# alvinwan/neural-backed-decision-trees

Measured on AMD Instinct MI355X. Metric: images/sec training SoftNBDT WRN28x10 CIFAR10, higher is better.
Workload: dtype bf16; 1 GPU; WideResNet-28-10 + SoftTreeSupLoss (induced-wrn28_10_cifar10, 10 leaves), CIFAR10-shaped 3x32x32, SGD m=0.9 wd=5e-4; batch_per_gpu=512, global_batch=512, parallelism=dp1

## Files before the change

### include/nbdt_hip.h

```cpp
#ifndef NBDT_HIP_H
#define NBDT_HIP_H

#include <stdint.h>

#ifdef __cplusplus
extern "C" {
#endif

#define NBDT_OK 0
#define NBDT_EINVAL (-1)
#define NBDT_EHIP (-2)
#define NBDT_ENOMEM (-3)

#define NBDT_F32 0
#define NBDT_BF16 1
#define NBDT_F16 2

const char* nbdt_last_error(void);
const char* nbdt_debug_last_igemm(void);
const char* nbdt_debug_last_igemm_full(void);
const char* nbdt_debug_last_wgrad(void);
int nbdt_version(void);
int nbdt_set_deterministic(int32_t on);
int nbdt_get_deterministic(void);
// ... 273 lines not shown
                         int32_t C, float* out, void* stream);
int nbdt_ref_bn_act_bwd(const float* gu, const float* gate, const float* gpool, const float* x, const float* save_mean,
                        const float* save_rstd, const float* gamma, const float* beta, int32_t act, const float* gx_add,
                        int32_t B, int32_t H, int32_t W, int32_t C, float* dsum, float* dgamma, float* dbeta, float* gx,
                        void* stream);
int nbdt_ref_dwconv_fwd(const float* x, const float* w, int32_t B, int32_t H, int32_t W, int32_t C, int32_t k,
                        int32_t stride, float* y, void* stream);
int nbdt_ref_dwconv_bwd_data(const float* gy, const float* w, int32_t B, int32_t H, int32_t W, int32_t C, int32_t k,
                             int32_t stride, float* gx, void* stream);
int nbdt_ref_dwconv_bwd_weight(const float* x, const float* gy, int32_t B, int32_t H, int32_t W, int32_t C, int32_t k,
                               int32_t stride, float* dw, void* stream);

int nbdt_stem_conv(const float* img, const float* w, int32_t B, int32_t H, int32_t W,
                   int32_t cout_real, int32_t cpad, int32_t stride, void* out, void* stream);
int nbdt_stem_wgrad(const float* img, const void* gy, int32_t B, int32_t H, int32_t W,
                    int32_t cout_real, int32_t cpad, int32_t stride, float* dw, void* stream);
int nbdt_linear_fwd(const float* x, const float* w, const float* b, int32_t B, int32_t K, int32_t N,
                    float* z, void* stream);
int nbdt_linear_bwd(const float* x, const float* w, const float* gz, int32_t B, int32_t K, int32_t N,
                    float* gx, float* gw, float* gb, void* stream);
int nbdt_sgd_step(float* p, float* g, float* buf, int64_t n, float lr, float momentum,
                  float weight_decay, float grad_scale, void* p_bf16, int32_t zero_grad, void* stream);

#define NBDT_U8 3
#define NBDT_AUGMENT_MAX_PAD 32
int nbdt_augment_batch(const void* src, int32_t src_dtype, const int64_t* labels_src, const int64_t* index, int32_t B,
                       int64_t N, int32_t H, int32_t W, int32_t pad, int32_t flip, const float* mean, const float* std,
                       const float* fill, uint64_t seed, uint64_t epoch, const int8_t* params_in, float* out,
                       int64_t* labels_out, int8_t* params_out, void* stream);

#define NBDT_RESIZED_CROP_RATIOS 4096
#define NBDT_RESIZED_CROP_ATTEMPTS 10
int nbdt_resized_crop_batch(const void* src, int32_t src_dtype, const int64_t* labels_src, const int64_t* index, int32_t B,
                            int64_t N, int32_t H, int32_t W, int32_t rs_h, int32_t rs_w, int32_t win_top, int32_t win_left,
                            int32_t out_h, int32_t out_w, int32_t flip, const float* mean, const float* std,
                            const double* scale, const double* ratio, const double* ratio_table, uint64_t seed,
                            uint64_t epoch, const int32_t* params_in, float* out, int64_t* labels_out, int32_t* params_out,
                            void* stream);
int nbdt_resized_crop_band_rows(int32_t H, int32_t W, int32_t rs_h, int32_t rs_w, int32_t win_top, int32_t win_left,
                                int32_t out_h, int32_t out_w);

int nbdt_augment_batch_sharded(const void* src, int32_t src_dtype, const int64_t* labels_src, const int64_t* index,
                               int64_t index_base, int32_t B, int64_t N, int32_t H, int32_t W, int32_t pad, int32_t flip,
                               const float* mean, const float* std, const float* fill, uint64_t seed, uint64_t epoch,
                               const int8_t* params_in, float* out, int64_t* labels_out, int8_t* params_out, void* stream);
int nbdt_resized_crop_batch_sharded(const void* src, int32_t src_dtype, const int64_t* labels_src, const int64_t* index,
// ... 26 lines not shown
```

### neural-backed-decision-trees_amd/csrc/common.h

```cpp
#pragma once
#include <hip/hip_runtime.h>
#include <hip/hip_bf16.h>
#include <hip/hip_fp16.h>
#include <stdint.h>
#include <stdio.h>
#include <string.h>

#include <mutex>

#include "../../include/nbdt_hip.h"

#if !defined(NBDT_TIMING_BUILD) &&                                                                                    \
    (defined(NBDT_EPI_TIMING) || (defined(NBDT_PP_TIMING) && (NBDT_PP_TIMING + 0) != 0) ||                            \
     (defined(NBDT_WPP_TIMING) && (NBDT_WPP_TIMING + 0) != 0) || (defined(NBDT_SEG_TIMING) && (NBDT_SEG_TIMING + 0) != 0) || \
     (defined(NBDT_RULES_TIMING) && (NBDT_RULES_TIMING + 0) != 0))
#error "timing switch without -DNBDT_TIMING_BUILD: a stamped build is not a product library (csrc/common.h)"
#endif
#ifdef NBDT_TIMING_BUILD
extern "C" __attribute__((weak, used, visibility("default"))) int nbdt_timing_build() { return 1; }
#endif

namespace nbdt {

extern thread_local char g_err[512];
// ... 43 lines not shown
bool wgrad_store_epilogue();
int reserved_cus();
float* det_rows(hipStream_t st, size_t floats);
const char* det_rows_why();
int det_fold(hipStream_t st, const float* rows, int nrows, size_t n, float* dst);

typedef unsigned short bf16_t;

__device__ __forceinline__ float bf16_to_f32(bf16_t v) {
  return __uint_as_float(((unsigned)v) << 16);
}
__device__ __forceinline__ bf16_t f32_to_bf16(float f) {
  unsigned u = __float_as_uint(f);
  if ((u & 0x7fffffffu) > 0x7f800000u) return (bf16_t)((u >> 16) | 0x40);
  u += 0x7fffu + ((u >> 16) & 1u);
  return (bf16_t)(u >> 16);
}
__device__ __forceinline__ unsigned pack_bf16x2(float lo, float hi) {
  unsigned r;
  asm("v_cvt_pk_bf16_f32 %0, %1, %2" : "=v"(r) : "v"(lo), "v"(hi));
  return r;
}

struct FastDiv {
  unsigned mul, sh, d;
};
inline FastDiv make_fastdiv(unsigned d) {
  FastDiv f;
  f.d = d;
  if (d == 1) { f.mul = 0; f.sh = 0; return f; }
  unsigned s = 0;
  while ((1ull << s) < d) ++s;
  const unsigned long long num = 1ull << (31 + s);
  f.mul = (unsigned)((num + d - 1) / d);
  f.sh = s - 1;
  return f;
}
__device__ __forceinline__ unsigned fdiv(unsigned n, const FastDiv& f) {
  return f.d == 1 ? n : (__umulhi(n, f.mul) >> f.sh);
}

struct PadGeom {
  int B, H, W, C;
  int npix;
  int row;
  int img;
// ... 119 lines not shown
```

### neural-backed-decision-trees_amd/csrc/conv.hip

```cpp
#include "common.h"
#include <stdlib.h>

using namespace nbdt;

static int check_desc(const nbdt_conv_desc* d);

static int conv_igemm_impl(const nbdt_conv_desc* d, const void* in, const void* w, void* out, const void* residual,
                           float* bn_scratch, void* stream, const nbdt::BnBwdArgs* bn = nullptr) {
  NBDT_REQUIRE(d && in && w && out, "null argument");
  int rc = check_desc(d);
  if (rc) return rc;
  const void* res = d->accumulate ? (const void*)out : residual;
  NBDT_REQUIRE(!(d->accumulate && residual), "accumulate and residual are exclusive");
  const int64_t M64 = (int64_t)d->B * d->gh * d->gw;
  NBDT_REQUIRE(M64 < (1ll << 31), "pixel grid too large");
  const int M = (int)M64;
  hipStream_t st = (hipStream_t)stream;
  nbdt::HaloGeom hg;
  if (nbdt::conv_halo_applicable(d, M, &hg))
    return nbdt::conv3x3_halo(d, hg, in, w, out, res, bn_scratch, bn, M, st);
  NBDT_REQUIRE(d->wide_tile != 2 && d->wide_tile != 4 && d->wide_tile != 5,
               "wide_tile = 2 / 4 / 5 (force 512-pixel tiles [with the padded LDS pitch] / half tiles): not a dense 3x3 stride-1 conv it fits");
  nbdt::g_last_igemm = "conv_igemm_dma_kernel";
  return nbdt::conv_igemm_dma(d, in, w, out, res, bn_scratch, bn, M, st);
// ... 72 lines not shown
  return conv_igemm_impl(d, in, w, out, residual, bn_scratch, stream);
}

extern "C" int nbdt_conv_igemm_bnbwd(const nbdt_conv_desc* d, const void* in, const void* w, void* out,
                                     const void* bn_x, const float* save_mean, const float* save_rstd,
                                     const float* gamma, const float* beta, float* bn_partials, void* stream) {
  NBDT_REQUIRE(bn_x && save_mean && save_rstd && gamma && beta && bn_partials, "null BatchNorm argument");
  NBDT_REQUIRE(d && !d->accumulate, "fused BatchNorm-backward sums are for plain outputs");
  nbdt::BnBwdArgs bn{bn_x, save_mean, save_rstd, gamma, beta};
  return conv_igemm_impl(d, in, w, out, nullptr, bn_partials, stream, &bn);
}

extern "C" int nbdt_conv_igemm_affine(const nbdt_conv_desc* d, const void* in, const void* w, void* out,
                                      const void* residual, const float* scale, const float* shift, int32_t act,
                                      void* stream) {
  NBDT_REQUIRE(scale && shift, "null scale / shift");
  NBDT_REQUIRE(act >= 0 && act <= 2, "unknown activation");
  NBDT_REQUIRE(d && !d->accumulate, "the fused inference epilogue is for plain outputs");
  nbdt::BnBwdArgs ep{nullptr, nullptr, nullptr, nullptr, nullptr};
  ep.aff_scale = scale; ep.aff_shift = shift; ep.aff_act = act;
  return conv_igemm_impl(d, in, w, out, residual, nullptr, stream, &ep);
}

__global__ __launch_bounds__(256) void weight_prep_kernel(const float* __restrict__ w, int cout, int taps,
                                                          int cin, bf16_t* __restrict__ wb,
                                                          bf16_t* __restrict__ wd) {
  const int64_t n = (int64_t)cout * taps * cin;
  for (int64_t i = (int64_t)blockIdx.x * 256 + threadIdx.x; i < n; i += (int64_t)gridDim.x * 256) {
    const bf16_t v = f32_to_bf16(w[i]);
    if (wb) wb[i] = v;
    if (wd) {
      const int ci = (int)(i % cin);
      const int64_t r = i / cin;
      const int t = (int)(r % taps);
      const int co = (int)(r / taps);
      wd[((int64_t)ci * taps + (taps - 1 - t)) * cout + co] = v;
    }
  }
}

__global__ __launch_bounds__(256) void weight_prep_batched_kernel(const float* __restrict__ flat,
                                                                  const long long* __restrict__ table, int n_layers,
                                                                  long long total_tiles, bf16_t* __restrict__ wd_flat) {
  __shared__ long long tab[64 * 6];
  __shared__ float tile[64][33];
  for (int i = threadIdx.x; i < n_layers * 6; i += 256) tab[i] = table[i];
  __syncthreads();
  const int tx = threadIdx.x & 31, ty = threadIdx.x >> 5;
  const int wx = threadIdx.x & 63, wy = threadIdx.x >> 6;
  for (long long e = blockIdx.x; e < total_tiles; e += gridDim.x) {
    int l = 0;
    while (l + 1 < n_layers && e >= tab[(l + 1) * 6 + 5]) ++l;
    const long long* T = tab + l * 6;
    const int cout = (int)T[2], taps = (int)T[3], cin = (int)T[4];
    const int cit = cin >> 5, cot = (cout + 63) >> 6;
    long long i = e - T[5];
    const int ci0 = (int)(i % cit) * 32;
    i /= cit;
    const int co0 = (int)(i % cot) * 64;
    const int t = (int)(i / cot);
    const float* src = flat + T[0];
    bf16_t* dst = wd_flat + T[1];
#pragma unroll
    for (int r = ty; r < 64; r += 8)
      tile[r][tx] = co0 + r < cout ? src[((long long)(co0 + r) * taps + t) * cin + ci0 + tx] : 0.f;
    __syncthreads();
#pragma unroll
    for (int r = wy; r < 32; r += 4)
      if (co0 + wx < cout)
        dst[((long long)(ci0 + r) * taps + (taps - 1 - t)) * cout + co0 + wx] = f32_to_bf16(tile[wx][r]);
    __syncthreads();
  }
}

extern "C" int nbdt_weight_prep_batched(const float* flat, const int64_t* table, int32_t n_layers, int64_t total_tiles,
                                        void* wd_flat, void* stream) {
  NBDT_REQUIRE(flat && table && wd_flat, "null argument");
  NBDT_REQUIRE(n_layers > 0 && n_layers <= 64 && total_tiles > 0, "bad layer table");
  long long blocks = total_tiles < 8192 ? total_tiles : 8192;
  hipLaunchKernelGGL(weight_prep_batched_kernel, dim3((unsigned)blocks), dim3(256), 0, (hipStream_t)stream, flat,
                     (const long long*)table, n_layers, (long long)total_tiles, (bf16_t*)wd_flat);
  NBDT_LAUNCH_CHECK();
  return NBDT_OK;
}

__global__ __launch_bounds__(256) void weight_tile_batched_kernel(const bf16_t* __restrict__ src,
                                                                  const long long* __restrict__ table, int n,
                                                                  long long total_tiles, bf16_t* __restrict__ dst) {
  __shared__ long long tab[64 * 5];
  for (int i = threadIdx.x; i < n * 5; i += 256) tab[i] = table[i];
  __syncthreads();
  for (long long e = blockIdx.x; e < total_tiles; e += gridDim.x) {
    int l = 0;
    while (l + 1 < n && e >= tab[(l + 1) * 5 + 4]) ++l;
    const long long* T = tab + l * 5;
    const int rows = (int)T[2], k = (int)T[3];
    const int nt32 = rows / 32;
    const int nt = nt32 % 5 == 0 ? 5 : (nt32 % 4 == 0 ? 4 : (nt32 % 2 == 0 ? 2 : 1));
    const int bn = 32 * nt, kchunks = k / 32;
    long long i = e - T[4];
    const int tap = (int)(i % 9);
    i /= 9;
    const int kc = (int)(i % kchunks);
    const int n_blk = (int)(i / kchunks);
    const bf16_t* s0 = src + T[0];
    bf16_t* d0 = dst + T[1] + (e - T[4]) * (long long)(bn * 32);
    for (int q = threadIdx.x; q < bn * 4; q += 256) {
      const int r = q >> 2, cp = q & 3;
      const int c = cp ^ ((r >> 2) & 3);
      const u32x4_t v = *(const u32x4_t*)(s0 + ((long long)(n_blk * bn + r) * 9 + tap) * k + kc * 32 + c * 8);
      *(u32x4_t*)(d0 + r * 32 + cp * 8) = v;
    }
  }
}

extern "C" int nbdt_weight_tile_batched(const void* src_bf16, const int64_t* table, int32_t n, int64_t total_tiles,
                                        void* dst_bf16, void* stream) {
  NBDT_REQUIRE(src_bf16 && table && dst_bf16, "null argument");
  NBDT_REQUIRE(n > 0 && n <= 64 && total_tiles > 0, "bad matrix table");
  long long blocks = total_tiles < 8192 ? total_tiles : 8192;
  hipLaunchKernelGGL(weight_tile_batched_kernel, dim3((unsigned)blocks), dim3(256), 0, (hipStream_t)stream,
                     (const bf16_t*)src_bf16, (const long long*)table, n, (long long)total_tiles, (bf16_t*)dst_bf16);
  NBDT_LAUNCH_CHECK();
  return NBDT_OK;
}

extern "C" int nbdt_weight_prep(const float* w, int32_t cout, int32_t taps, int32_t cin, void* w_bf16,
                                void* wd_bf16, void* stream) {
  NBDT_REQUIRE(w && (w_bf16 || wd_bf16), "null argument");
  NBDT_REQUIRE(cout > 0 && taps > 0 && cin > 0, "bad shape");
  const int64_t n = (int64_t)cout * taps * cin;
  const int grid = (int)((n + 255) / 256 < 2048 ? (n + 255) / 256 : 2048);
  hipLaunchKernelGGL(weight_prep_kernel, dim3(grid), dim3(256), 0, (hipStream_t)stream, w, cout, taps, cin,
                     (bf16_t*)w_bf16, (bf16_t*)wd_bf16);
  NBDT_LAUNCH_CHECK();
  return NBDT_OK;
}
```

### neural-backed-decision-trees_amd/csrc/misc.hip

```cpp
#include "common.h"

#include <atomic>
#include <map>
#include <utility>

using namespace nbdt;

namespace nbdt {
static std::atomic<int> g_deterministic{0};
bool deterministic() { return g_deterministic.load(std::memory_order_relaxed) != 0; }

struct DetBuf { float* ptr = nullptr; size_t floats = 0; bool captured = false; };
static std::mutex g_det_mutex;
static std::map<std::pair<int, hipStream_t>, DetBuf> g_det_bufs;

static thread_local char g_det_why[200] = "";
const char* det_rows_why() { return g_det_why; }

float* det_rows(hipStream_t st, size_t floats) {
  int dev = 0;
  snprintf(g_det_why, sizeof(g_det_why), "hipMalloc / hipGetDevice failed");
  if (hipGetDevice(&dev) != hipSuccess) return nullptr;
  std::lock_guard<std::mutex> lock(g_det_mutex);
  DetBuf& b = g_det_bufs[std::make_pair(dev, st)];
// ... 468 lines not shown
    const long long n = (long long)B * K;
    hipLaunchKernelGGL(linear_bwd_x_kernel, dim3((unsigned)((n + 255) / 256)), dim3(256), 0, st, gz, w, B, K, N, gx);
    NBDT_LAUNCH_CHECK();
  }
  if (gw) {
    const long long n = (long long)N * (K + 1);
    const int splits = (B >= 64 && !deterministic()) ? 16 : 1;
    const int bpb = (B + splits - 1) / splits;
    hipLaunchKernelGGL(linear_bwd_w_kernel, dim3((unsigned)((n + 255) / 256), (B + bpb - 1) / bpb), dim3(256), 0, st, gz,
                       x, B, K, N, bpb, gw, gb);
    NBDT_LAUNCH_CHECK();
  }
  return NBDT_OK;
}

__global__ __launch_bounds__(256) void sgd_kernel(float* __restrict__ p, float* __restrict__ g,
                                                  float* __restrict__ buf, long long n, float lr, float momentum,
                                                  float wd, float gscale, bf16_t* __restrict__ pb, int zero_g) {
  const long long n4 = n >> 2;
  for (long long i = (long long)blockIdx.x * 256 + threadIdx.x; i < n4; i += (long long)gridDim.x * 256) {
    float4 pv = ((const float4*)p)[i];
    const float4 gv = ((const float4*)g)[i];
    float4 bv = ((const float4*)buf)[i];
    bv.x = momentum * bv.x + (gscale * gv.x + wd * pv.x);
    bv.y = momentum * bv.y + (gscale * gv.y + wd * pv.y);
    bv.z = momentum * bv.z + (gscale * gv.z + wd * pv.z);
    bv.w = momentum * bv.w + (gscale * gv.w + wd * pv.w);
    pv.x -= lr * bv.x; pv.y -= lr * bv.y; pv.z -= lr * bv.z; pv.w -= lr * bv.w;
    ((float4*)buf)[i] = bv;
    ((float4*)p)[i] = pv;
    if (zero_g) ((float4*)g)[i] = float4{0.f, 0.f, 0.f, 0.f};
    if (pb) {
      uint2 o;
      o.x = pack_bf16x2(pv.x, pv.y);
      o.y = pack_bf16x2(pv.z, pv.w);
      ((uint2*)pb)[i] = o;
    }
  }
  if (blockIdx.x == 0 && threadIdx.x < (n & 3)) {
    const long long i = (n4 << 2) + threadIdx.x;
    const float b = momentum * buf[i] + (gscale * g[i] + wd * p[i]);
    buf[i] = b;
    p[i] -= lr * b;
    if (zero_g) g[i] = 0.f;
    if (pb) pb[i] = f32_to_bf16(p[i]);
  }
}

extern "C" int nbdt_sgd_step(float* p, float* g, float* buf, int64_t n, float lr, float momentum,
                             float weight_decay, float grad_scale, void* p_bf16, int32_t zero_grad, void* stream) {
  NBDT_REQUIRE(p && g && buf && n > 0, "bad sgd arguments");
// ... 12 lines not shown
```

### neural-backed-decision-trees_amd/csrc/rules.hip

```cpp
#include "common.h"

#include <algorithm>
#include <vector>

namespace nbdt {
thread_local char g_err[512] = "";
}

using namespace nbdt;

struct nbdt_tree {
  int device;
  int cus;
  int C, N, R, L, root, max_depth;
  int sched_len;
  int32_t* d_all;
  const int32_t *node_off, *slot_off, *slot_cls, *cls_off, *cls_slot, *slot_next;
  const int32_t* sched;
};

struct TreeView {
  int C, N, R, L, root, max_depth, sched_len;
  int tl_ints;
  int staged;
// ... 1254 lines not shown
      if (want_scores) {
        a.scores[sample * 3] = h_net;
        a.scores[sample * 3 + 1] = top_diff;
        a.scores[sample * 3 + 2] = spread;
      }
    }
    __syncthreads();
  }

  if (a.node_counts != nullptr)
    for (int i = threadIdx.x; i < 5 * t.N; i += (int)blockDim.x)
      if (cnt[i] != 0) add_i64(a.node_counts + i, cnt[i]);
  if (a.totals != nullptr && threadIdx.x < 4 && tot[threadIdx.x] != 0) add_i64(a.totals + threadIdx.x, tot[threadIdx.x]);
  if (a.first_error != nullptr)
    for (int i = threadIdx.x; i <= t.max_depth; i += (int)blockDim.x)
      if (fed[i] != 0) add_i64(a.first_error + i, fed[i]);
  if (a.node_entropy != nullptr)
    for (int i = threadIdx.x; i < 2 * t.N; i += (int)blockDim.x)
      if (ent[i] != 0ull) add_i64(a.node_entropy + i, (long long)ent[i]);
}


extern "C" const char* nbdt_last_error(void) { return nbdt::g_err; }
extern "C" int nbdt_version(void) { return 116; }
extern "C" int nbdt_device_count(void) {
  int n = 0;
  if (hipGetDeviceCount(&n) != hipSuccess) return 0;
  return n;
}

static int pick_tps(int C, int R) { return (C <= 64 && R <= 64) ? 64 : (C <= 512 && R <= 512) ? 256 : 1024; }

static void build_slot_schedule(int R, const int32_t* slot_off, int lanes, std::vector<int32_t>* out, int* len) {
  std::vector<int> order(R);
  for (int s = 0; s < R; ++s) order[s] = s;
  auto length = [&](int s) { return slot_off[s + 1] - slot_off[s]; };
  std::stable_sort(order.begin(), order.end(), [&](int a, int b) { return length(a) > length(b); });
  const int waves = lanes / 64, chunks = (R + 63) / 64;
  std::vector<std::vector<int>> mine(waves);
  std::vector<long> load(waves, 0);
  for (int c = 0; c < chunks; ++c) {
    const int longest = length(order[c * 64]);
    int w = 0;
    for (int i = 1; i < waves; ++i)
      if (load[i] < load[w]) w = i;
    mine[w].push_back(c);
    load[w] += 64 + 8L * longest;
// ... 375 lines not shown
```

### neural-backed-decision-trees_amd/nbdt/_C.py

```python
import ctypes
import os
from ctypes import POINTER, c_char_p, c_float, c_int, c_int32, c_int64, c_void_p

import numpy as np
import torch

_LIBPATH = os.environ.get("NBDT_HIP_LIB") or os.path.join(os.path.dirname(os.path.abspath(__file__)), "_lib",
                                                         "libnbdt_hip.so")
_lib = None

NBDT_F32, NBDT_BF16, NBDT_F16 = 0, 1, 2
NBDT_U8 = 3
NBDT_AUGMENT_MAX_PAD = 32
NBDT_RESIZED_CROP_RATIOS = 4096
NBDT_RESIZED_CROP_ATTEMPTS = 10
_ZTYPE = {torch.float32: NBDT_F32, torch.bfloat16: NBDT_BF16, torch.float16: NBDT_F16}


class NBDTHipError(RuntimeError):
    pass


class ConvDesc(ctypes.Structure):
    _fields_ = [
# ... 166 lines not shown
                                 _P, _P, _P]),
    "nbdt_se_param_grad": (c_int, [_P, _P, _P, _P, c_int32, c_int32, c_int32, c_int32, _P, _P, _P, _P, _P]),
    "nbdt_dropout_fwd": (c_int, [_P, c_int64, c_float, ctypes.c_uint32, _P, _P, _P]),
    "nbdt_dropout_bwd": (c_int, [_P, c_int64, c_float, _P, _P, _P]),
    "nbdt_augment_batch": (c_int, [_P, c_int32, _P, _P, c_int32, c_int64, c_int32, c_int32, c_int32, c_int32,
                                   POINTER(c_float), POINTER(c_float), POINTER(c_float), ctypes.c_uint64, ctypes.c_uint64,
                                   _P, _P, _P, _P, _P]),
    "nbdt_resized_crop_batch": (c_int, [_P, c_int32, _P, _P, c_int32, c_int64] + [c_int32] * 9 +
                                [POINTER(c_float), POINTER(c_float), POINTER(ctypes.c_double), POINTER(ctypes.c_double), _P,
                                 ctypes.c_uint64, ctypes.c_uint64, _P, _P, _P, _P, _P]),
    "nbdt_resized_crop_band_rows": (c_int, [c_int32] * 8),
    "nbdt_augment_batch_sharded": (c_int, [_P, c_int32, _P, _P, c_int64, c_int32, c_int64, c_int32, c_int32, c_int32, c_int32,
                                           POINTER(c_float), POINTER(c_float), POINTER(c_float), ctypes.c_uint64,
                                           ctypes.c_uint64, _P, _P, _P, _P, _P]),
    "nbdt_resized_crop_batch_sharded": (c_int, [_P, c_int32, _P, _P, c_int64, c_int32, c_int64] + [c_int32] * 9 +
                                        [POINTER(c_float), POINTER(c_float), POINTER(ctypes.c_double),
                                         POINTER(ctypes.c_double), _P, ctypes.c_uint64, ctypes.c_uint64, _P, _P, _P, _P, _P]),
    "nbdt_stem_patches": (c_int, [_P, c_int32, c_int32, c_int32, c_int32, c_int32, c_int32, c_int32, _P, _P]),
    "nbdt_maxpool3x3s2_fwd": (c_int, [_P, c_int32, c_int32, c_int32, c_int32, c_int32, _P, _P, _P]),
    "nbdt_maxpool3x3s2_bwd": (c_int, [_P, _P, c_int32, c_int32, c_int32, c_int32, c_int32, _P, _P]),
    "nbdt_linear_fwd": (c_int, [_P, _P, _P, c_int32, c_int32, c_int32, _P, _P]),
    "nbdt_linear_bwd": (c_int, [_P, _P, _P, c_int32, c_int32, c_int32, _P, _P, _P, _P]),
    "nbdt_sgd_step": (c_int, [_P, _P, _P, c_int64, c_float, c_float, c_float, c_float, _P, c_int32, _P]),
}


def _missing(name):
    def raiser(*_a, **_k):
        raise NBDTHipError(f"{_LIBPATH} does not export {name}: stale build, re-run build()")
    return raiser


def exported_symbols():
    l = ctypes.CDLL(_LIBPATH)
    return [n for n in SIGNATURES if hasattr(l, n)]


def lib():
    global _lib
    if _lib is None:
        if not os.path.exists(_LIBPATH):
            raise NBDTHipError(
                f"{_LIBPATH} is missing: build it with `python __graft_entry__.py build` "
                "(hipcc --offload-arch=gfx950).  There is no CPU fallback for the NBDT hot path.")
        l = ctypes.CDLL(_LIBPATH)
        if hasattr(l, "nbdt_timing_build") and os.environ.get("NBDT_ALLOW_TIMING_BUILD") != "1":
            raise NBDTHipError(f"{_LIBPATH} is a timing build (exports nbdt_timing_build): its kernels carry "
# ... 221 lines not shown
```

### neural-backed-decision-trees_amd/nbdt/engine.py

```python
import math

import torch

from nbdt import _C, ops

ALIGN = 8

_SIDE_STREAMS = {}


def side_stream(device):
    dev = torch.device(device)
    key = (dev.type, dev.index if dev.index is not None else torch.cuda.current_device())
    if key not in _SIDE_STREAMS:
        _SIDE_STREAMS[key] = torch.cuda.Stream(device=dev)
    return _SIDE_STREAMS[key]


def _pad32(c):
    return (c + 31) // 32 * 32


class ParamStore:

# ... 297 lines not shown
        self.training = True
        self.act_dtype = torch.bfloat16
        self.debug_keep = False
        self.debug_share_serial = False
        self.fuse_stats = True
        self.fuse_eval = True
        self.share_bn2_tensors, self.share_bn1_tensors = 5, 6
        self.fuse_bn1_bwd = True
        self._side = None
        self._cu_share = None
        self._share_join = False
        self._share_split = (False, 250.0)
        self._share_calibrated = True
        self.cu_share_report = None
        self._overlap = True
        self._seg_ops = {}
        self._seg_skip = set()
        self.share_stage_us = {}
        self._slot_pairs = {}
        self._slot_arena, self._slot_arena_pairs = None, 0
        self._partials = None
        self._reserved_now = 0
        self._grad_is_zero = False
        self._B = None

    def seg_op(self, key, build, sources, sources32, on_side=False):
        op = self._seg_ops.get(key)
        if op is None:
            op = SegOp(build(), sources, sources32, on_side)
            if self.act_dtype != torch.float32:
                if on_side and self._side is not None and self._overlap:
                    self._side.wait_stream(torch.cuda.current_stream(self.device))
                    with torch.cuda.stream(self._side):
                        op.retile()
                    torch.cuda.current_stream(self.device).wait_stream(self._side)
                else:
                    op.retile()
            self._seg_ops[key] = op
        return op

    def _retile_seg(self, on_side):
        if self.act_dtype == torch.float32:
            return
        for op in self._seg_ops.values():
            if op.on_side == on_side:
                op.retile()
# ... 218 lines not shown

    def _pool_head(self, x, mean, rstd, gamma, beta, head):
        B = self._B
        self._pooled = self._tensor("pooled", (B, self.feat_c))
        ops.bn_relu_pool(x, mean, rstd, gamma, beta, self._pooled)
        if not head:
            return self._pooled
        z = self._tensor("z", (B, self.num_classes))
        w, b = self.classifier_names
        ops.linear_fwd(self._pooled, self.store.p(w), self.store.p(b), z)
        return z

    def _head_backward(self, gz, gpooled):
        if gpooled is not None:
            return gpooled
        gz = gz.contiguous()
        gpool = self._tensor("gpool", (self._B, self.feat_c))
        w, b = self.classifier_names
        ops.linear_bwd(self._pooled, self.store.p(w), gz, gpool, self.store.g(w), self.store.g(b))
        return gpool

    def _begin_backward(self, comm):
        self._grad_is_zero = False
        self.join_side_stream()
        if self._cu_share is not None and not self._share_calibrated:
            self.calibrate_cu_share(comm)
        self.reset_slot_pairs()

    def _units_backward(self, units, comm):
        main = torch.cuda.current_stream(self.device)
        two_streams = self._side is not None and self._overlap
        if two_streams:
            self._side.wait_stream(main)
        buckets = self.grad_buckets() if comm is not None else None
        side_mark = None
        for i, u in enumerate(reversed(units)):
            if two_streams:
                if side_mark is not None:
                    main.wait_event(side_mark)
                side_mark = torch.cuda.Event()
                side_mark.record(self._side)
            yield i, u
            if comm is not None and u["key"] in self.bucket_units:
                self.join_side_stream()
                comm.reduce_range(self.store.grad, *buckets[self.bucket_units.index(u["key"])])
                self._reserve_for(comm)

# ... 29 lines not shown
            self._wt_dgrad = torch.empty(n_el, dtype=torch.bfloat16, device=self.device)
            frows, drows, off, tf, td = [], [], 0, 0, 0

            def ntile(r):
                r32 = r // 32
                return 5 if r32 % 5 == 0 else 4 if r32 % 4 == 0 else 2 if r32 % 2 == 0 else 1

            wd_off = {}
            o = 0
            for c in self.convs:
                wd_off[c.name] = o
                o += c.numel()
            for c in dense:
                frows.append([self.store.entries[c.name][0], off, c.cout, c.cin, tf])
                drows.append([wd_off[c.name], off, c.cin, c.cout, td])
                c.wt_fwd = self._wt_fwd[off:off + c.numel()]
                c.wt_dgrad = self._wt_dgrad[off:off + c.numel()]
                off += c.numel()
                tf += (c.cout // (32 * ntile(c.cout))) * (c.cin // 32) * 9
                td += (c.cin // (32 * ntile(c.cin))) * (c.cout // 32) * 9
            self._wt_ftable = torch.tensor(frows, dtype=torch.int64, device=self.device)
            self._wt_dtable = torch.tensor(drows, dtype=torch.int64, device=self.device)
            self._wt_ftotal, self._wt_dtotal = tf, td
        self.refresh_derived_weights()

    def refresh_derived_weights(self):
        for b in self.bns:
            b._affine = None
        if self.act_dtype == torch.float32:
            for c in self.convs:
                c.wd32 = self.store.p(c.name).flip(1).permute(2, 1, 0).contiguous()
        if self._wt_n:
            ops.weight_tile_batched(self.store.bf16, self._wt_ftable, self._wt_n, self._wt_ftotal, self._wt_fwd)
        self._retile_seg(False)
        if self._side is None or not self._overlap:
            ops.weight_prep_batched(self.store.flat, self._wd_table, len(self.convs), self._wd_total, self._wd_flat)
            if self._wt_n:
                ops.weight_tile_batched(self._wd_flat, self._wt_dtable, self._wt_n, self._wt_dtotal, self._wt_dgrad)
            self._retile_seg(True)
            return
        self._side.wait_stream(torch.cuda.current_stream(self.device))
        with torch.cuda.stream(self._side):
            ops.weight_prep_batched(self.store.flat, self._wd_table, len(self.convs), self._wd_total, self._wd_flat)
            if self._wt_n:
                ops.weight_tile_batched(self._wd_flat, self._wt_dtable, self._wt_n, self._wt_dtotal, self._wt_dgrad)
            self._retile_seg(True)

    def sgd_step(self, lr, momentum=0.9, weight_decay=5e-4, grad_scale=1.0, zero_grad=False):
        self.join_side_stream()
        s = self.store
        ops.sgd_step(s.flat, s.grad, s.mom, lr, momentum, weight_decay, grad_scale, s.bf16, zero_grad=zero_grad)
        self._grad_is_zero = bool(zero_grad)
        self.refresh_derived_weights()

    def zero_grad(self):
        if not self._grad_is_zero:
            self.store.zero_grad()
        self._grad_is_zero = False

    def extra_param_views(self, buf):
        return {}

    def named_params(self, which="flat"):
        buf = {"flat": self.store.flat, "grad": self.store.grad, "bf16": self.store.bf16}[which]
        out = dict(self.extra_param_views(buf))
        for c in self.convs:
            out[c.name] = c.logical(buf)
        for b in self.bns:
            out[b.name + ".weight"] = self.store._view(buf, b.name + ".weight")[:b.c_real]
            out[b.name + ".bias"] = self.store._view(buf, b.name + ".bias")[:b.c_real]
        return out

    def named_buffers(self):
# ... 707 lines not shown
```

### neural-backed-decision-trees_amd/nbdt/ops.py

```python
import ctypes

import torch

from nbdt import _C
from nbdt._C import ConvDesc, WgradDesc, check, lib, ptr

BN_SLOTS = 32
BN_EPS = 1e-5
BN_MOMENTUM = 0.1


def set_deterministic(on):
    check(lib().nbdt_set_deterministic(1 if on else 0))


def is_deterministic():
    return bool(lib().nbdt_get_deterministic())


def set_wgrad_store_epilogue(on):
    check(lib().nbdt_set_wgrad_store_epilogue(1 if on else 0))


def wgrad_store_epilogue():
# ... 612 lines not shown
            raise _C.NBDTHipError(f"unknown statistic {name!r}; nbdt_tree_stats has {', '.join(STATS_FIELDS)}")
        if t is None:
            continue
        if t.dtype != torch.int64 or t.device != z.device or not t.is_contiguous() or t.numel() != sizes[name]:
            raise _C.NBDTHipError(f"{name}: expected a contiguous int64 tensor of {sizes[name]} elements on {z.device}, "
                                  f"got {t.dtype} {tuple(t.shape)} on {t.device}")
        setattr(block, name, t.data_ptr())
    if y is not None:
        if y.is_floating_point() or y.dim() != 1 or y.shape[0] != B:
            raise _C.NBDTHipError(f"tree_stats_accumulate takes class-index labels [B], got {y.dtype} {tuple(y.shape)}")
        y = y.to(device=z.device, dtype=torch.int64).contiguous()
    if scores is not None and (scores.dtype != torch.float32 or scores.device != z.device or not scores.is_contiguous()
                               or tuple(scores.shape) != (B, 3)):
        raise _C.NBDTHipError(f"scores: expected a contiguous fp32 [{B}, 3] tensor on {z.device}")
    check(lib().nbdt_tree_stats_accumulate(handle.h, ptr(z), _C.ztype_of(z), B, ld, ptr(y), ctypes.byref(block),
                                           ptr(scores), _C.stream_of(z)))


def sgd_step(p, g, buf, lr, momentum, weight_decay, grad_scale=1.0, p_bf16=None, zero_grad=False):
    check(lib().nbdt_sgd_step(ptr(p), ptr(g), ptr(buf), p.numel(), lr, momentum, weight_decay, grad_scale,
                              ptr(p_bf16), 1 if zero_grad else 0, stream_ptr(p.device)))



ACT_NONE, ACT_RELU, ACT_SWISH = 0, 1, 2


def bn_act_apply(x, mean, rstd, gamma, beta, y, act=ACT_SWISH, gate=None, residual=None):
    B, H, W, C = _dims(x)
    if _ref(x):
        check(lib().nbdt_ref_bn_act_apply(ptr(x), ptr(mean), ptr(rstd), ptr(gamma), ptr(beta), act, ptr(gate),
                                          ptr(residual), B, H, W, C, ptr(y), stream_ptr(x.device)))
        return
    check(lib().nbdt_bn_act_apply(ptr(x), ptr(mean), ptr(rstd), ptr(gamma), ptr(beta), act, ptr(gate),
                                  ptr(residual), B, H, W, C, ptr(y), stream_ptr(x.device)))


def bn_act_pool(x, mean, rstd, gamma, beta, out, act=ACT_SWISH, mul=None, scale=None):
    B, H, W, C = _dims(x)
    scale = 1.0 / (H * W) if scale is None else scale
    if _ref(x):
        check(lib().nbdt_ref_bn_act_pool(ptr(x), ptr(mean), ptr(rstd), ptr(gamma), ptr(beta), act, ptr(mul), scale,
                                         B, H, W, C, ptr(out), stream_ptr(x.device)))
        return
    check(lib().nbdt_bn_act_pool(ptr(x), ptr(mean), ptr(rstd), ptr(gamma), ptr(beta), act, ptr(mul), scale,
                                 B, H, W, C, ptr(out), stream_ptr(x.device)))
# ... 301 lines not shown
```

Before: 31610 images/sec.

## Fuse SGD update with bf16 cast and derived conv weight re-tiling

Measured after the change: 31730 images/sec (median of 6 runs). About the same (+0.4%).

```diff
diff --git a/include/nbdt_hip.h b/include/nbdt_hip.h
--- a/include/nbdt_hip.h
+++ b/include/nbdt_hip.h
@@ -319,6 +319,18 @@
 int nbdt_sgd_step(float* p, float* g, float* buf, int64_t n, float lr, float momentum,
                   float weight_decay, float grad_scale, void* p_bf16, int32_t zero_grad, void* stream);
 
+#define NBDT_SGD_FUSED_MAX_LAYERS 64
+#define NBDT_SGD_FUSED_MAX_RANGES 128
+#define NBDT_SGD_FUSED_CHUNK 2048
+#ifndef NBDT_SGD_FUSED_PATCH_CIN
+#define NBDT_SGD_FUSED_PATCH_CIN 64
+#endif
+int nbdt_sgd_fused_step(float* p, float* g, float* buf, int64_t n, float lr, float momentum,
+                        float weight_decay, float grad_scale, int32_t zero_grad, void* p_bf16,
+                        void* wt_fwd, void* wt_dgrad, int64_t wt_elems, void* wd_flat, int64_t wd_elems,
+                        const int64_t* table_host, const int64_t* table_dev, int32_t n_layers,
+                        int32_t n_ranges, void* stream);
+
 #define NBDT_U8 3
 #define NBDT_AUGMENT_MAX_PAD 32
 int nbdt_augment_batch(const void* src, int32_t src_dtype, const int64_t* labels_src, const int64_t* index, int32_t B,
diff --git a/neural-backed-decision-trees_amd/csrc/common.h b/neural-backed-decision-trees_amd/csrc/common.h
--- a/neural-backed-decision-trees_amd/csrc/common.h
+++ b/neural-backed-decision-trees_amd/csrc/common.h
@@ -89,6 +89,12 @@
   return r;
 }
 
+__device__ __forceinline__ void sgd_update(float& p, float g, float& b, float lr, float momentum, float wd,
+                                           float gscale) {
+  b = momentum * b + (gscale * g + wd * p);
+  p -= lr * b;
+}
+
 struct FastDiv {
   unsigned mul, sh, d;
 };
diff --git a/neural-backed-decision-trees_amd/csrc/conv.hip b/neural-backed-decision-trees_amd/csrc/conv.hip
--- a/neural-backed-decision-trees_amd/csrc/conv.hip
+++ b/neural-backed-decision-trees_amd/csrc/conv.hip
@@ -118,6 +118,31 @@
   return conv_igemm_impl(d, in, w, out, residual, nullptr, stream, &ep);
 }
 
+
+__device__ __forceinline__ long long wd_index(int taps, int cout, int ci, int t, int co) {
+  return ((long long)ci * taps + (taps - 1 - t)) * cout + co;
+}
+__device__ __forceinline__ void wprep_patch(unsigned i, int cout, int cin, int cw, int* ci0, int* co0, int* t) {
+  const unsigned cit = (unsigned)((cin + cw - 1) / cw), cot = (unsigned)((cout + 63) >> 6);
+  *ci0 = (int)(i % cit) * cw;
+  i /= cit;
+  *co0 = (int)(i % cot) * 64;
+  *t = (int)(i / cot);
+}
+__device__ __forceinline__ int wtile_nt(int rows) {
+  const int nt32 = rows / 32;
+  return nt32 % 5 == 0 ? 5 : (nt32 % 4 == 0 ? 4 : (nt32 % 2 == 0 ? 2 : 1));
+}
+__device__ __forceinline__ int wtile_swz(int r, int c) { return c ^ ((r >> 2) & 3); }
+__device__ __forceinline__ long long wtile_base(int bn, int kchunks, int n_blk, int kc, int tap) {
+  return ((long long)(n_blk * kchunks + kc) * 9 + tap) * (long long)(bn * 32);
+}
+__device__ __forceinline__ long long wtile_chunk(int rows, int k, int row, int tap, int kc, int c) {
+  const int bn = 32 * wtile_nt(rows);
+  const int r = row % bn;
+  return wtile_base(bn, k / 32, row / bn, kc, tap) + r * 32 + wtile_swz(r, c) * 8;
+}
+
 __global__ __launch_bounds__(256) void weight_prep_kernel(const float* __restrict__ w, int cout, int taps,
                                                           int cin, bf16_t* __restrict__ wb,
                                                           bf16_t* __restrict__ wd) {
@@ -130,7 +155,7 @@
       const int64_t r = i / cin;
       const int t = (int)(r % taps);
       const int co = (int)(r / taps);
-      wd[((int64_t)ci * taps + (taps - 1 - t)) * cout + co] = v;
+      wd[wd_index(taps, cout, ci, t, co)] = v;
     }
   }
 }
@@ -149,12 +174,8 @@
     while (l + 1 < n_layers && e >= tab[(l + 1) * 6 + 5]) ++l;
     const long long* T = tab + l * 6;
     const int cout = (int)T[2], taps = (int)T[3], cin = (int)T[4];
-    const int cit = cin >> 5, cot = (cout + 63) >> 6;
-    long long i = e - T[5];
-    const int ci0 = (int)(i % cit) * 32;
-    i /= cit;
-    const int co0 = (int)(i % cot) * 64;
-    const int t = (int)(i / cot);
+    int ci0, co0, t;
+    wprep_patch((unsigned)(e - T[5]), cout, cin, 32, &ci0, &co0, &t);
     const float* src = flat + T[0];
     bf16_t* dst = wd_flat + T[1];
 #pragma unroll
@@ -164,7 +185,7 @@
 #pragma unroll
     for (int r = wy; r < 32; r += 4)
       if (co0 + wx < cout)
-        dst[((long long)(ci0 + r) * taps + (taps - 1 - t)) * cout + co0 + wx] = f32_to_bf16(tile[wx][r]);
+        dst[wd_index(taps, cout, ci0 + r, t, co0 + wx)] = f32_to_bf16(tile[wx][r]);
     __syncthreads();
   }
 }
@@ -191,19 +212,17 @@
     while (l + 1 < n && e >= tab[(l + 1) * 5 + 4]) ++l;
     const long long* T = tab + l * 5;
     const int rows = (int)T[2], k = (int)T[3];
-    const int nt32 = rows / 32;
-    const int nt = nt32 % 5 == 0 ? 5 : (nt32 % 4 == 0 ? 4 : (nt32 % 2 == 0 ? 2 : 1));
-    const int bn = 32 * nt, kchunks = k / 32;
+    const int bn = 32 * wtile_nt(rows), kchunks = k / 32;
     long long i = e - T[4];
     const int tap = (int)(i % 9);
     i /= 9;
     const int kc = (int)(i % kchunks);
     const int n_blk = (int)(i / kchunks);
     const bf16_t* s0 = src + T[0];
-    bf16_t* d0 = dst + T[1] + (e - T[4]) * (long long)(bn * 32);
+    bf16_t* d0 = dst + T[1] + wtile_base(bn, kchunks, n_blk, kc, tap);
     for (int q = threadIdx.x; q < bn * 4; q += 256) {
       const int r = q >> 2, cp = q & 3;
-      const int c = cp ^ ((r >> 2) & 3);
+      const int c = wtile_swz(r, cp);
       const u32x4_t v = *(const u32x4_t*)(s0 + ((long long)(n_blk * bn + r) * 9 + tap) * k + kc * 32 + c * 8);
       *(u32x4_t*)(d0 + r * 32 + cp * 8) = v;
     }
@@ -232,3 +251,183 @@
   NBDT_LAUNCH_CHECK();
   return NBDT_OK;
 }
+
+
+constexpr int kFusedCin = NBDT_SGD_FUSED_PATCH_CIN;
+static_assert(kFusedCin == 32 || kFusedCin == 64, "the patch is 32 or 64 input channels wide");
+
+struct SgdFusedArgs {
+  float *p, *g, *m;
+  bf16_t *pb, *wt_fwd, *wd_flat, *wt_dgrad;
+  const long long* table;
+  int n_layers, n_ranges;
+  long long conv_items, total_items;
+  float lr, momentum, wd, gscale;
+  int zero_g;
+};
+
+__device__ __forceinline__ uint2 sgd_fused_quad(const SgdFusedArgs& a, long long i, float4 pv, const float4 gv, float4 bv) {
+  sgd_update(pv.x, gv.x, bv.x, a.lr, a.momentum, a.wd, a.gscale);
+  sgd_update(pv.y, gv.y, bv.y, a.lr, a.momentum, a.wd, a.gscale);
+  sgd_update(pv.z, gv.z, bv.z, a.lr, a.momentum, a.wd, a.gscale);
+  sgd_update(pv.w, gv.w, bv.w, a.lr, a.momentum, a.wd, a.gscale);
+  *(float4*)(a.m + i) = bv;
+  *(float4*)(a.p + i) = pv;
+  if (a.zero_g) *(float4*)(a.g + i) = float4{0.f, 0.f, 0.f, 0.f};
+  uint2 o;
+  o.x = pack_bf16x2(pv.x, pv.y);
+  o.y = pack_bf16x2(pv.z, pv.w);
+  *(uint2*)(a.pb + i) = o;
+  return o;
+}
+
+__global__ __launch_bounds__(256) void sgd_fused_kernel(const SgdFusedArgs a) {
+  constexpr int LPR = kFusedCin / 4;
+  constexpr int RPP = 256 / LPR;
+  constexpr int NP = 64 / RPP;
+  __shared__ long long tab[NBDT_SGD_FUSED_MAX_LAYERS * 8 + NBDT_SGD_FUSED_MAX_RANGES * 4];
+  __shared__ __attribute__((aligned(16))) bf16_t img[kFusedCin][72];
+  for (int i = threadIdx.x; i < a.n_layers * 8 + a.n_ranges * 4; i += 256) tab[i] = a.table[i];
+  __syncthreads();
+  const long long* rtab = tab + a.n_layers * 8;
+  const int q = threadIdx.x % LPR, row = threadIdx.x / LPR;
+  for (long long e = blockIdx.x; e < a.total_items; e += gridDim.x) {
+    if (e >= a.conv_items) {
+      int j = 0;
+      while (j + 1 < a.n_ranges && e >= rtab[(j + 1) * 4 + 2]) ++j;
+      const long long* R = rtab + j * 4;
+      const long long lo = R[0] + (e - R[2]) * NBDT_SGD_FUSED_CHUNK, end = R[0] + R[1];
+      const long long hi = lo + NBDT_SGD_FUSED_CHUNK < end ? lo + NBDT_SGD_FUSED_CHUNK : end;
+      for (long long i = lo + 4 * threadIdx.x; i < hi; i += 1024) {
+        if (i + 4 <= hi) {
+          sgd_fused_quad(a, i, *(const float4*)(a.p + i), *(const float4*)(a.g + i), *(const float4*)(a.m + i));
+          continue;
+        }
+        for (long long k = i; k < hi; ++k) {
+          float pv = a.p[k], bv = a.m[k];
+          sgd_update(pv, a.g[k], bv, a.lr, a.momentum, a.wd, a.gscale);
+          a.m[k] = bv;
+          a.p[k] = pv;
+          if (a.zero_g) a.g[k] = 0.f;
+          a.pb[k] = f32_to_bf16(pv);
+        }
+      }
+      continue;
+    }
+    int l = 0;
+    while (l + 1 < a.n_layers && e >= tab[(l + 1) * 8 + 5]) ++l;
+    const long long* T = tab + l * 8;
+    const int cout = (int)T[2], taps = (int)T[3], cin = (int)T[4];
+    const long long wt_off = T[6];
+    int ci0, co0, t;
+    wprep_patch((unsigned)(e - T[5]), cout, cin, kFusedCin, &ci0, &co0, &t);
+    const int ci = ci0 + 4 * q;
+    long long idx[NP];
+    float4 pv[NP], gv[NP], bv[NP];
+#pragma unroll
+    for (int h = 0; h < NP; ++h) {
+      const int co = co0 + row + RPP * h;
+      idx[h] = co < cout && ci < cin ? T[0] + ((long long)co * taps + t) * cin + ci : -1;
+      if (idx[h] >= 0) {
+        pv[h] = *(const float4*)(a.p + idx[h]);
+        gv[h] = *(const float4*)(a.g + idx[h]);
+        bv[h] = *(const float4*)(a.m + idx[h]);
+      }
+    }
+#pragma unroll
+    for (int h = 0; h < NP; ++h) {
+      if (idx[h] < 0) continue;
+      const int r = row + RPP * h;
+      const uint2 o = sgd_fused_quad(a, idx[h], pv[h], gv[h], bv[h]);
+      if (wt_off >= 0)
+        *(uint2*)(a.wt_fwd + wt_off + wtile_chunk(cout, cin, co0 + r, t, ci >> 5, (ci & 31) >> 3) + (q & 1) * 4) = o;
+      img[4 * q + 0][r] = (bf16_t)(o.x & 0xffffu);
+      img[4 * q + 1][r] = (bf16_t)(o.x >> 16);
+      img[4 * q + 2][r] = (bf16_t)(o.y & 0xffffu);
+      img[4 * q + 3][r] = (bf16_t)(o.y >> 16);
+    }
+    __syncthreads();
+#pragma unroll
+    for (int it = threadIdx.x; it < kFusedCin * 8; it += 256) {
+      const int r2 = it >> 3, q2 = it & 7;
+      if (ci0 + r2 >= cin || co0 + 8 * q2 >= cout) continue;
+      const u32x4_t v = *(const u32x4_t*)&img[r2][8 * q2];
+      *(u32x4_t*)(a.wd_flat + T[1] + wd_index(taps, cout, ci0 + r2, t, co0 + 8 * q2)) = v;
+      if (wt_off >= 0)
+        *(u32x4_t*)(a.wt_dgrad + wt_off + wtile_chunk(cin, cout, ci0 + r2, taps - 1 - t, (co0 + 8 * q2) >> 5, q2 & 3)) = v;
+    }
+    __syncthreads();
+  }
+}
+
+extern "C" int nbdt_sgd_fused_step(float* p, float* g, float* buf, int64_t n, float lr, float momentum,
+                                   float weight_decay, float grad_scale, int32_t zero_grad, void* p_bf16,
+                                   void* wt_fwd, void* wt_dgrad, int64_t wt_elems, void* wd_flat, int64_t wd_elems,
+                                   const int64_t* table_host, const int64_t* table_dev, int32_t n_layers,
+                                   int32_t n_ranges, void* stream) {
+  NBDT_REQUIRE(p && g && buf && p_bf16 && table_host && table_dev && n > 0, "null argument");
+  NBDT_REQUIRE(n_layers >= 0 && n_layers <= NBDT_SGD_FUSED_MAX_LAYERS && n_ranges >= 0 &&
+               n_ranges <= NBDT_SGD_FUSED_MAX_RANGES && n_layers + n_ranges > 0, "bad table size");
+  NBDT_REQUIRE(wt_elems >= 0 && wd_elems >= 0 && (n_layers == 0 || wd_flat), "bad derived-weight buffers");
+  const uintptr_t bits = (uintptr_t)p | (uintptr_t)g | (uintptr_t)buf | (uintptr_t)p_bf16 | (uintptr_t)wt_fwd |
+                         (uintptr_t)wt_dgrad | (uintptr_t)wd_flat;
+  NBDT_REQUIRE((bits % 16) == 0, "flat buffers must be 16-byte aligned");
+  int64_t span[NBDT_SGD_FUSED_MAX_LAYERS + NBDT_SGD_FUSED_MAX_RANGES][2];
+  int64_t items = 0;
+  for (int l = 0; l < n_layers; ++l) {
+    const int64_t* T = table_host + l * 8;
+    const int64_t cout = T[2], taps = T[3], cin = T[4];
+    NBDT_REQUIRE(cout > 0 && cout % 32 == 0 && cout < (1 << 20) && cin > 0 && cin % 32 == 0 && cin < (1 << 20) &&
+                 taps >= 1 && taps <= 64, "layer shape: cout and cin multiples of 32, 1 to 64 taps");
+    const int64_t numel = cout * taps * cin;
+    NBDT_REQUIRE(T[0] >= 0 && T[0] % 8 == 0 && T[0] <= n - numel, "layer outside the flat store or misaligned");
+    NBDT_REQUIRE(T[1] >= 0 && T[1] % 8 == 0 && T[1] <= wd_elems - numel, "layer outside the data-gradient copy");
+    NBDT_REQUIRE(T[6] == -1 || (taps == 9 && wt_fwd && wt_dgrad && T[6] >= 0 && T[6] % 8 == 0 && T[6] <= wt_elems - numel),
+                 "tiles: 3x3 layers only, inside both tile buffers");
+    NBDT_REQUIRE(T[5] == items && T[7] == 0, "layer table: wrong first item");
+    for (int o = 0; o < l; ++o) {
+      const int64_t* U = table_host + o * 8;
+      const int64_t un = U[2] * U[3] * U[4];
+      NBDT_REQUIRE(T[1] + numel <= U[1] || U[1] + un <= T[1], "layers overlap in the data-gradient copy");
+      NBDT_REQUIRE(T[6] < 0 || U[6] < 0 || T[6] + numel <= U[6] || U[6] + un <= T[6], "layers overlap in the tile buffers");
+    }
+    span[l][0] = T[0];
+    span[l][1] = numel;
+    items += taps * ((cout + 63) / 64) * ((cin + kFusedCin - 1) / kFusedCin);
+  }
+  const int64_t conv_items = items;
+  for (int r = 0; r < n_ranges; ++r) {
+    const int64_t* R = table_host + n_layers * 8 + r * 4;
+    NBDT_REQUIRE(R[0] >= 0 && R[0] % 4 == 0 && R[1] > 0 && R[0] <= n - R[1], "range outside the flat store or misaligned");
+    NBDT_REQUIRE(R[2] == items && R[3] == 0, "range table: wrong first item");
+    span[n_layers + r][0] = R[0];
+    span[n_layers + r][1] = R[1];
+    items += (R[1] + NBDT_SGD_FUSED_CHUNK - 1) / NBDT_SGD_FUSED_CHUNK;
+  }
+  const int ns = n_layers + n_ranges;
+  for (int i = 1; i < ns; ++i) {
+    const int64_t s0 = span[i][0], s1 = span[i][1];
+    int j = i;
+    for (; j > 0 && span[j - 1][0] > s0; --j) { span[j][0] = span[j - 1][0]; span[j][1] = span[j - 1][1]; }
+    span[j][0] = s0;
+    span[j][1] = s1;
+  }
+  int64_t at = 0;
+  for (int i = 0; i < ns; ++i) {
+    NBDT_REQUIRE(span[i][0] == at, "layers and ranges must cover the flat store exactly once (overlap or gap)");
+    at += span[i][1];
+  }
+  NBDT_REQUIRE(at == n, "layers and ranges must cover the flat store exactly once (short of its end)");
+  SgdFusedArgs a;
+  a.p = p; a.g = g; a.m = buf;
+  a.pb = (bf16_t*)p_bf16; a.wt_fwd = (bf16_t*)wt_fwd; a.wd_flat = (bf16_t*)wd_flat; a.wt_dgrad = (bf16_t*)wt_dgrad;
+  a.table = (const long long*)table_dev;
+  a.n_layers = n_layers; a.n_ranges = n_ranges;
+  a.conv_items = conv_items; a.total_items = items;
+  a.lr = lr; a.momentum = momentum; a.wd = weight_decay; a.gscale = grad_scale;
+  a.zero_g = zero_grad ? 1 : 0;
+  const long long blocks = items < 8192 ? items : 8192;
+  hipLaunchKernelGGL(sgd_fused_kernel, dim3((unsigned)blocks), dim3(256), 0, (hipStream_t)stream, a);
+  NBDT_LAUNCH_CHECK();
+  return NBDT_OK;
+}
diff --git a/neural-backed-decision-trees_amd/csrc/misc.hip b/neural-backed-decision-trees_amd/csrc/misc.hip
--- a/neural-backed-decision-trees_amd/csrc/misc.hip
+++ b/neural-backed-decision-trees_amd/csrc/misc.hip
@@ -514,11 +514,10 @@
     float4 pv = ((const float4*)p)[i];
     const float4 gv = ((const float4*)g)[i];
     float4 bv = ((const float4*)buf)[i];
-    bv.x = momentum * bv.x + (gscale * gv.x + wd * pv.x);
-    bv.y = momentum * bv.y + (gscale * gv.y + wd * pv.y);
-    bv.z = momentum * bv.z + (gscale * gv.z + wd * pv.z);
-    bv.w = momentum * bv.w + (gscale * gv.w + wd * pv.w);
-    pv.x -= lr * bv.x; pv.y -= lr * bv.y; pv.z -= lr * bv.z; pv.w -= lr * bv.w;
+    sgd_update(pv.x, gv.x, bv.x, lr, momentum, wd, gscale);
+    sgd_update(pv.y, gv.y, bv.y, lr, momentum, wd, gscale);
+    sgd_update(pv.z, gv.z, bv.z, lr, momentum, wd, gscale);
+    sgd_update(pv.w, gv.w, bv.w, lr, momentum, wd, gscale);
     ((float4*)buf)[i] = bv;
     ((float4*)p)[i] = pv;
     if (zero_g) ((float4*)g)[i] = float4{0.f, 0.f, 0.f, 0.f};
diff --git a/neural-backed-decision-trees_amd/csrc/rules.hip b/neural-backed-decision-trees_amd/csrc/rules.hip
--- a/neural-backed-decision-trees_amd/csrc/rules.hip
+++ b/neural-backed-decision-trees_amd/csrc/rules.hip
@@ -1300,7 +1300,7 @@
 
 
 extern "C" const char* nbdt_last_error(void) { return nbdt::g_err; }
-extern "C" int nbdt_version(void) { return 116; }
+extern "C" int nbdt_version(void) { return 117; }
 extern "C" int nbdt_device_count(void) {
   int n = 0;
   if (hipGetDeviceCount(&n) != hipSuccess) return 0;
diff --git a/neural-backed-decision-trees_amd/nbdt/_C.py b/neural-backed-decision-trees_amd/nbdt/_C.py
--- a/neural-backed-decision-trees_amd/nbdt/_C.py
+++ b/neural-backed-decision-trees_amd/nbdt/_C.py
@@ -212,7 +212,11 @@
     "nbdt_linear_fwd": (c_int, [_P, _P, _P, c_int32, c_int32, c_int32, _P, _P]),
     "nbdt_linear_bwd": (c_int, [_P, _P, _P, c_int32, c_int32, c_int32, _P, _P, _P, _P]),
     "nbdt_sgd_step": (c_int, [_P, _P, _P, c_int64, c_float, c_float, c_float, c_float, _P, c_int32, _P]),
+    "nbdt_sgd_fused_step": (c_int, [_P, _P, _P, c_int64, c_float, c_float, c_float, c_float, c_int32, _P, _P, _P, c_int64,
+                                    _P, c_int64, _P, _P, c_int32, c_int32, _P]),
 }
+
+NBDT_SGD_FUSED_MAX_LAYERS, NBDT_SGD_FUSED_MAX_RANGES, NBDT_SGD_FUSED_CHUNK, NBDT_SGD_FUSED_PATCH_CIN = 64, 128, 2048, 64
 
 
 def _missing(name):
diff --git a/neural-backed-decision-trees_amd/nbdt/engine.py b/neural-backed-decision-trees_amd/nbdt/engine.py
--- a/neural-backed-decision-trees_amd/nbdt/engine.py
+++ b/neural-backed-decision-trees_amd/nbdt/engine.py
@@ -343,6 +343,9 @@
         self._partials = None
         self._reserved_now = 0
         self._grad_is_zero = False
+        self.fused_optimizer = True
+        self._fused = None
+        self._derived_on_side = False
         self._B = None
 
     def seg_op(self, key, build, sources, sources32, on_side=False):
@@ -607,7 +610,9 @@
 
     def _begin_backward(self, comm):
         self._grad_is_zero = False
-        self.join_side_stream()
+        if self._derived_on_side:
+            self.join_side_stream()
+            self._derived_on_side = False
         if self._cu_share is not None and not self._share_calibrated:
             self.calibrate_cu_share(comm)
         self.reset_slot_pairs()
@@ -683,7 +688,27 @@
             self._wt_ftable = torch.tensor(frows, dtype=torch.int64, device=self.device)
             self._wt_dtable = torch.tensor(drows, dtype=torch.int64, device=self.device)
             self._wt_ftotal, self._wt_dtotal = tf, td
+        self._fused = self._fused_optimizer_table()
         self.refresh_derived_weights()
+
+    def _fused_optimizer_table(self):
+        wd_off, wt_off, o = {}, {}, 0
+        for c in self.convs:
+            wd_off[c.name] = o
+            o += c.numel()
+        o = 0
+        for c in self.convs:
+            if c.k == 3 and c.stride == 1:
+                wt_off[c.name] = o
+                o += c.numel()
+        layers = [(self.store.entries[c.name][0], wd_off[c.name], c.cout, c.taps, c.cin, wt_off.get(c.name, -1))
+                  for c in self.convs]
+        if not layers or len(layers) > _C.NBDT_SGD_FUSED_MAX_LAYERS:
+            return None
+        table, n_layers, n_ranges = ops.sgd_fused_table(self.store.flat.numel(), layers)
+        if n_ranges > _C.NBDT_SGD_FUSED_MAX_RANGES:
+            return None
+        return table, table.to(self.device), n_layers, n_ranges
 
     def refresh_derived_weights(self):
         for b in self.bns:
@@ -701,6 +726,7 @@
             self._retile_seg(True)
             return
         self._side.wait_stream(torch.cuda.current_stream(self.device))
+        self._derived_on_side = True
         with torch.cuda.stream(self._side):
             ops.weight_prep_batched(self.store.flat, self._wd_table, len(self.convs), self._wd_total, self._wd_flat)
             if self._wt_n:
@@ -710,6 +736,17 @@
     def sgd_step(self, lr, momentum=0.9, weight_decay=5e-4, grad_scale=1.0, zero_grad=False):
         self.join_side_stream()
         s = self.store
+        if self.fused_optimizer and self._fused is not None and self.act_dtype != torch.float32:
+            table, table_dev, n_layers, n_ranges = self._fused
+            wt_fwd, wt_dgrad = (self._wt_fwd, self._wt_dgrad) if self._wt_n else (None, None)
+            ops.sgd_fused_step(s.flat, s.grad, s.mom, lr, momentum, weight_decay, grad_scale, zero_grad, s.bf16, wt_fwd,
+                               wt_dgrad, self._wd_flat, table, table_dev, n_layers, n_ranges)
+            self._grad_is_zero = bool(zero_grad)
+            for b in self.bns:
+                b._affine = None
+            self._retile_seg(False)
+            self._retile_seg(True)
+            return
         ops.sgd_step(s.flat, s.grad, s.mom, lr, momentum, weight_decay, grad_scale, s.bf16, zero_grad=zero_grad)
         self._grad_is_zero = bool(zero_grad)
         self.refresh_derived_weights()
diff --git a/neural-backed-decision-trees_amd/nbdt/ops.py b/neural-backed-decision-trees_amd/nbdt/ops.py
--- a/neural-backed-decision-trees_amd/nbdt/ops.py
+++ b/neural-backed-decision-trees_amd/nbdt/ops.py
@@ -658,6 +658,42 @@
                               ptr(p_bf16), 1 if zero_grad else 0, stream_ptr(p.device)))
 
 
+def sgd_fused_table(n, layers):
+    rows, items = [], 0
+    for (p_off, wd_off, cout, taps, cin, wt_off) in layers:
+        rows += [p_off, wd_off, cout, taps, cin, items, wt_off, 0]
+        items += taps * ((cout + 63) // 64) * ((cin + _C.NBDT_SGD_FUSED_PATCH_CIN - 1) // _C.NBDT_SGD_FUSED_PATCH_CIN)
+    ranges, at = [], 0
+    for p_off, numel in sorted((l[0], l[2] * l[3] * l[4]) for l in layers):
+        assert p_off >= at, "convolution weights overlap in the flat store"
+        if p_off > at:
+            ranges.append((at, p_off - at))
+        at = p_off + numel
+    assert at <= n, "a convolution weight ends past the flat store"
+    if at < n:
+        ranges.append((at, n - at))
+    for start, length in ranges:
+        rows += [start, length, items, 0]
+        items += (length + _C.NBDT_SGD_FUSED_CHUNK - 1) // _C.NBDT_SGD_FUSED_CHUNK
+    spans = sorted([(l[0], l[2] * l[3] * l[4]) for l in layers] + ranges)
+    at = 0
+    for start, length in spans:
+        assert start == at and length > 0, "the fused optimizer's table does not tile the flat store"
+        at += length
+    assert at == n, "the fused optimizer's table does not tile the flat store"
+    return torch.tensor(rows, dtype=torch.int64), len(layers), len(ranges)
+
+
+def sgd_fused_step(p, g, buf, lr, momentum, weight_decay, grad_scale, zero_grad, p_bf16, wt_fwd, wt_dgrad, wd_flat,
+                   table_host, table_dev, n_layers, n_ranges):
+    assert table_host.device.type == "cpu" and table_host.dtype == torch.int64 and table_host.is_contiguous()
+    check(lib().nbdt_sgd_fused_step(ptr(p), ptr(g), ptr(buf), p.numel(), lr, momentum, weight_decay, grad_scale,
+                                    1 if zero_grad else 0, ptr(p_bf16), ptr(wt_fwd), ptr(wt_dgrad),
+                                    0 if wt_fwd is None else wt_fwd.numel(), ptr(wd_flat),
+                                    0 if wd_flat is None else wd_flat.numel(), table_host.data_ptr(), ptr(table_dev),
+                                    n_layers, n_ranges, stream_ptr(p.device)))
+
+
 
 ACT_NONE, ACT_RELU, ACT_SWISH = 0, 1, 2
 
```
